# leodd/Lifted-Hybrid-Variational-Inference

Hardware: AMD Instinct MI355X
Metric: lbp_sweeps_per_sec_10M_edge_hybrid_mrf (higher is better)
Workload: dtype f64

## Files before the change

include/lhvi.h:

```cpp
#ifndef LHVI_H
#define LHVI_H

#include <stddef.h>
#include <stdint.h>

#ifdef __cplusplus
extern "C" {
#endif

#define LHVI_ABI_VERSION 26
#define LHVI_MAX_ARITY 6

#define LHVI_OK 0
#define LHVI_E_ARG (-1)
#define LHVI_E_LAUNCH (-2)
#define LHVI_E_UNSUPPORTED (-3)
#define LHVI_E_NODEVICE (-4)
#define LHVI_E_NOT_PD (-5)

#define LHVI_POT_GENERIC 0
#define LHVI_POT_TABLE 1
#define LHVI_POT_GAUSSIAN 2
#define LHVI_POT_QUADRATIC 3
#define LHVI_POT_HYBRID_QUADRATIC 4
#define LHVI_POT_LINEAR_GAUSSIAN 5
#define LHVI_POT_X2 6
#define LHVI_POT_XY 7
#define LHVI_POT_MLN 8
#define LHVI_POT_MLN_HARD 9
#define LHVI_POT_IMAGE_NODE 10
#define LHVI_POT_IMAGE_EDGE 11

typedef struct lhvi_graph {
    int32_t V, F, E, nnz;
    const int32_t* fac_ptr;
    const int32_t* edge_var;
    const int32_t* edge_fac;
    const int32_t* edge_canon;
    const int32_t* var_ptr;
    const int32_t* var_edge;
    const double* edge_count;
    const int32_t* fac_pot;
    const double* var_value;
    const int32_t* var_dom;
    const double* var_mult;
    const double* fac_mult;
    int32_t D;
    const int32_t* dom_cont;
    const double* dom_lo;
    const double* dom_hi;
    const int32_t* dom_ptr;
    const double* dom_val;
    const double* edge_value;
    const int32_t* slot_var;
    const int32_t* hub_vars;
    int32_t n_hubs;
} lhvi_graph_t;
#define LHVI_HUB_DEGREE 64

typedef struct lhvi_pots {
    int32_t P;
    const int32_t* kind;
    const int32_t* off;
    const double* param;
    int32_t interpreted;
} lhvi_pots_t;

int lhvi_version(void);
const char* lhvi_strerror(int code);
int lhvi_last_hip_error(void);
int lhvi_device_count(void);


int lhvi_gabp_init(const lhvi_graph_t* g, double* f2v, double* v2f, void* stream);
int lhvi_gabp_v2f(const lhvi_graph_t* g, const double* f2v, double* v2f, void* stream);
int lhvi_gabp_f2v(const lhvi_graph_t* g, const lhvi_pots_t* pots, const double* v2f, double* f2v, void* stream);
int lhvi_gabp_run(const lhvi_graph_t* g, const lhvi_pots_t* pots, double* f2v, double* v2f, int iterations, void* stream);
typedef struct lhvi_gabp_plan {
    const int32_t* pslot;
    const int32_t* info;
    const double* count;
    int32_t n_hub_rows;
    const int32_t* rec;
    const double* pot_words;
    const int32_t* seg;
    int32_t n_seg;
} lhvi_gabp_plan_t;
size_t lhvi_gabp_pull_workspace_bytes(const lhvi_graph_t* g);
int lhvi_gabp_pull(const lhvi_graph_t* g, const lhvi_pots_t* pots, const lhvi_gabp_plan_t* plan, const double* v_prev,
                   double* v_next, int first, void* stream);
int lhvi_gabp_run_pull(const lhvi_graph_t* g, const lhvi_pots_t* pots, const lhvi_gabp_plan_t* plan, double* f2v, double* v2f,
                       int iterations, void* ws, size_t ws_bytes, void* stream);

int lhvi_gabp_graph_create(const lhvi_graph_t* g, const lhvi_pots_t* pots, const lhvi_gabp_plan_t* plan, double* f2v, double* v2f,
                           double* mu_var, int iterations, void* ws, size_t ws_bytes, void** handle_out);
int lhvi_gabp_graph_launch(void* handle, void* stream);
int lhvi_gabp_graph_destroy(void* handle);

int lhvi_gabp_marginals(const lhvi_graph_t* g, const double* f2v, double* mu_var, void* stream);

size_t lhvi_log_likelihood_workspace_bytes(const lhvi_graph_t* g);
int lhvi_log_likelihood(const lhvi_graph_t* g, const lhvi_pots_t* pots, const double* x, double* out, void* ws, size_t ws_bytes,
                        void* stream);


#define LHVI_PBP_EP 1u
#define LHVI_PBP_EPBP_DISCRETE 2u
#define LHVI_PBP_SKIP_TERMS 16u
#define LHVI_PBP_LEAVE_ROOM 256u
#define LHVI_PBP_CQ 512u
#define LHVI_PBP_BOUNDARY_TOTALS 2048u
#define LHVI_PBP_NO_UNIQ 4096u
#define LHVI_PBP_V2F_RECORDS 8192u
#define LHVI_PBP_WIDE_PAIRS 16384u
#define LHVI_PBP_SHARE_CUS 32768u
#define LHVI_PBP_NO_GRID 128u
#define LHVI_PBP_FUSED_RECORDS16 131072u
#define LHVI_PBP_F2V_HEAVY 262144u
#define LHVI_PBP_F2V_SMALL 524288u
#define LHVI_PBP_F2V_PAIR 1048576u
#define LHVI_PBP_F2V_FAST 2097152u
#define LHVI_PBP_F2V_CQ 4194304u
#define LHVI_PBP_F2V_GENERIC 8388608u
#define LHVI_PBP_F2V_ALL (LHVI_PBP_F2V_HEAVY | LHVI_PBP_F2V_SMALL | LHVI_PBP_F2V_PAIR | LHVI_PBP_F2V_FAST | LHVI_PBP_F2V_CQ | LHVI_PBP_F2V_GENERIC)
#define LHVI_PBP_POW2_GROUPS 65536u

typedef struct lhvi_pbp {
    int32_t n;
    int32_t T;
    uint32_t flags;
    double var_threshold;
    double max_log_value;
    const double* particles;
    const double* old_particles;
    const int32_t* np;
    const uint8_t* uniq;
    const double* q;
    const int32_t* fast_edges;
    int32_t n_fast;
    const int32_t* generic_edges;
    int32_t n_generic;
    int32_t generic_pts_log2;
    const void* fast_desc;
    const void* heavy_desc;
    int32_t n_heavy;
    const void* light_desc;
    int32_t n_light;
    const int32_t* bslot;
    const int32_t* brow_ptr;
    const int64_t* brow_off;
    const int32_t* brow_peer;
    const double* recv;
    int32_t rank;
    const double* var_degree;
    int32_t var_lo, var_hi;
    uint32_t* f2v_ticket;
    const int32_t* prop_desc;
    int32_t n_prop_desc;
    const void* pair_desc;
    int32_t n_pair;
    const void* cq_desc;
    int32_t n_cq;
    const int32_t* v2f_wide;
    int32_t n_v2f_wide;
    const int32_t* v2f_narrow;
    int32_t n_v2f_narrow;
    const int32_t* v2f_hub;
    int32_t n_v2f_hub;
    const int32_t* v2f_mid16;
    int32_t n_v2f_mid16;
    const int32_t* v2f_mid32;
    int32_t n_v2f_mid32;
    const int32_t* prop_hub;
    int32_t n_prop_hub;
    double* prop_partial;
    const int32_t* resample_vars;
    int32_t n_resample_vars;
    const void* small16_desc;
    int32_t n_small16;
    const void* small32_desc;
    int32_t n_small32;
    const int64_t* halo_off;
    double* halo_buf;
} lhvi_pbp_t;

#define LHVI_PBP_DESC_BYTES 128
#define LHVI_PBP_TICKET_WORDS 16
#define LHVI_PBP_TICKET_COUNTERS 8
int lhvi_pbp_describe(const lhvi_graph_t* g, const lhvi_pots_t* pots, const lhvi_pbp_t* s, const int32_t* edges, int32_t count,
                      void* desc_out, void* stream);
int lhvi_pbp_describe_cq(const lhvi_graph_t* g, const lhvi_pots_t* pots, const lhvi_pbp_t* s, const int32_t* edges, int32_t count,
                         void* desc_out, void* stream);
int lhvi_pbp_var_sum(const lhvi_graph_t* g, const lhvi_pbp_t* s, const double* f2v, double* out, void* stream);
int lhvi_pbp_domain_grid(const lhvi_graph_t* g, const lhvi_pbp_t* s, double* x, void* stream);
int lhvi_pbp_refine_grid(const lhvi_graph_t* g, const lhvi_pbp_t* s, const double* logb, double* x, double* best, double* best_val,
                         void* stream);
int lhvi_debug_exp(const double* x, double* y, int64_t n, void* stream);
int lhvi_debug_exp_acc(const double* x, const double* c, double* y, int64_t n, void* stream);
int lhvi_debug_exp_acc_floor(const double* x, const double* c, double* y, int64_t n, void* stream);
int lhvi_debug_log(const double* x, double* y, int64_t n, int32_t which, void* stream);

int lhvi_pbp_classify(const lhvi_graph_t* g, const lhvi_pots_t* pots, const lhvi_pbp_t* s, uint8_t* edge_class, void* stream);

int lhvi_pbp_uniq(const lhvi_graph_t* g, int32_t n, const double* particles, const int32_t* np, uint8_t* uniq, void* stream);
int lhvi_pbp_v2f(const lhvi_graph_t* g, const lhvi_pbp_t* s, const double* f2v, double* v2f, void* stream);
int lhvi_pbp_f2v(const lhvi_graph_t* g, const lhvi_pots_t* pots, const lhvi_pbp_t* s, const double* v2f, double* f2v, void* stream);
int lhvi_pbp_proposal(const lhvi_graph_t* g, const lhvi_pbp_t* s, const double* f2v, double* eta, double* q, void* stream);
int lhvi_pbp_proposal_partial(const lhvi_graph_t* g, const lhvi_pbp_t* s, const double* f2v, double* eta, double* ph, void* stream);
int lhvi_pbp_proposal_finish(const lhvi_graph_t* g, const lhvi_pbp_t* s, const double* ph, double* q, void* stream);
int lhvi_pbp_boundary_pack(const lhvi_graph_t* g, const lhvi_pbp_t* s, const double* f2v, const double* ph, int32_t nb,
                           const int32_t* bvars, double* send, void* stream);
int lhvi_pbp_boundary_reduce(int32_t n_items, const int32_t* width, const int32_t* src_ptr, const int64_t* src_off,
                             const int32_t* dst_ptr, const int64_t* dst_off, const double* in, double* out, void* stream);
int lhvi_pbp_init(const lhvi_graph_t* g, const lhvi_pbp_t* s, double* eta, double* q, double* f2v, double* v2f, void* stream);
int lhvi_pbp_resample(const lhvi_graph_t* g, const lhvi_pbp_t* s, const int64_t* var_gid, uint64_t seed, uint32_t iteration, double* particles_out, void* stream);
int lhvi_pbp_edge_points(const lhvi_graph_t* g, const lhvi_pots_t* pots, const lhvi_pbp_t* s, const double* v2f,
                         int32_t nq, const int32_t* qedge, int32_t npts, const double* x, double* out, void* stream);
int lhvi_pbp_resample_uniq(const lhvi_graph_t* g, const lhvi_pbp_t* s, const int64_t* var_gid, uint64_t seed, uint32_t iteration,
                           double* particles_out, uint8_t* uniq_out, void* stream);
int lhvi_pbp_belief_points(const lhvi_graph_t* g, const lhvi_pots_t* pots, const lhvi_pbp_t* s, const double* v2f,
                           int32_t nq, const int32_t* qvar, int32_t npts, const double* x, double* out, void* stream);
int lhvi_pbp_var_fused(const lhvi_graph_t* g, const lhvi_pbp_t* s, const double* f2v, double* v2f, double* eta, double* q,
                       const int64_t* var_gid, uint64_t seed, uint32_t iteration, double* particles_out, uint8_t* uniq_out,
                       const int32_t* desc, int32_t n16, int32_t n32_t32, int32_t n32_t64, void* stream);
int lhvi_pbp_var_fused64(const lhvi_graph_t* g, const lhvi_pbp_t* s, const double* f2v, double* v2f, double* eta, double* q,
                         const int64_t* var_gid, uint64_t seed, uint32_t iteration, double* particles_out, uint8_t* uniq_out,
                         const int32_t* desc, int32_t n64_t32, int32_t n64_t64, void* stream);
int lhvi_pbp_quad(const lhvi_graph_t* g, const lhvi_pots_t* pots, const lhvi_pbp_t* s, const double* v2f, int64_t nq,
                  const int32_t* row_var, const int64_t* qptr, const int32_t* qedge, const double* qmult, const double* lo,
                  const double* hi, double epsabs, double epsrel, double* z, double* abserr, int32_t* status, void* stream);
int lhvi_pbp_map_brent(const lhvi_graph_t* g, const lhvi_pots_t* pots, const lhvi_pbp_t* s, const double* v2f, int64_t nq,
                       const int32_t* row_var, const int64_t* qptr, const int32_t* qedge, const double* qmult, double xtol,
                       int32_t maxfun, double* xout, double* fout, int32_t* nfev, void* stream);
int lhvi_pbp_kl(const lhvi_graph_t* g, const lhvi_pots_t* pots, const lhvi_pbp_t* s, const double* v2f, int64_t nq,
                const int32_t* row_var, const int64_t* qptr, const int32_t* qedge, const double* qmult, const double* logz,
                int32_t Kp, const double* wp, const double* mup, const double* varp, const double* a, const double* b,
                double epsabs, double epsrel, double* kl, double* abserr, int32_t* status, int32_t* neval, void* stream);

int lhvi_pbp_halo_pack(const double* v2f, int32_t n, int32_t n_rows, const int32_t* row_edge, const int64_t* row_off,
                       const int32_t* row_width, const double* q, int32_t n_q, const int32_t* q_var, const int64_t* q_off,
                       double* out, void* stream);
int lhvi_pbp_halo_unpack(const double* in, int32_t n, int32_t n_rows, const int32_t* row_edge, const int64_t* row_off,
                         const int32_t* row_width, double* v2f, int32_t n_q, const int32_t* q_var, const int64_t* q_off,
                         double* q, void* stream);


typedef struct lhvi_vi {
    int32_t K;
    int32_t T;
    int32_t Dmax;
    int32_t quirks;
    const double* gh_x;
    const double* gh_w;
    const double* w;
    const double* eta_c;
    const double* eta_d;
    const double* obs_var;
    const double* var_N;
    const int32_t* fac_list;
    int32_t n_cc, n_grp3, n_grp6, n_rest3, n_rest6;
    int32_t n_tiny;
    int32_t tiny_par_words;
    const int32_t* edge_axis;
} lhvi_vi_t;
#define LHVI_VI_GAUSSIAN_PDF 2
#define LHVI_VI_GROUP_SLOTS 24
#define LHVI_VI_GROUP_COMP 48
#define LHVI_VI_TINY_NODES 32

// ... 273 lines not shown
```

lifted-hybrid-variational-inference_amd/csrc/pbp.hip:

```cpp
#include "common.hpp"
#include "potential.hpp"
#include "fastmath.hpp"
#include "cq.hpp"
#include "gk21.hpp"

namespace lhvi {

__device__ __forceinline__ double wave_sum(double v) { return dpp_wave_reduce(v, SumOp()); }
__device__ __forceinline__ double wave_max(double v) { return dpp_wave_reduce(v, MaxOp()); }
__device__ __forceinline__ int wave_sum_i(int v) {
#pragma unroll
    for (int off = 32; off > 0; off >>= 1) v += __shfl_xor(v, off);
    return v;
}

constexpr double PAD_LOG_TERM = -6.0e5;

__host__ __device__ __forceinline__ int var_first(const lhvi_pbp_t& s) { return s.var_hi > s.var_lo ? s.var_lo : 0; }
__host__ __device__ __forceinline__ int var_limit(const lhvi_graph_t& g, const lhvi_pbp_t& s) { return s.var_hi > s.var_lo ? s.var_hi : g.V; }

__device__ __forceinline__ double norm_pdf_std(double x, double mu, double sig) {
    const double u = (x - mu) / sig;
    return exp(-u * u * 0.5) / (2.506628274631 * sig);
}
// ... 739 lines not shown
        item = nxt;
    }
};

struct HeavyData { double y, m, x0, x1; };

#ifndef LHVI_HEAVY_BLOCK
#define LHVI_HEAVY_BLOCK 256
#endif
#ifndef LHVI_HEAVY_WAVES
#define LHVI_HEAVY_WAVES 7
#endif
#ifndef LHVI_HEAVY_UNROLL
#define LHVI_HEAVY_UNROLL 4
#endif
constexpr int HEAVY_BLOCK = LHVI_HEAVY_BLOCK;

template <int CTRL, int BANK>
__device__ __forceinline__ double dpp_into(double old, double src) {
    const int lo = __builtin_amdgcn_update_dpp(__double2loint(old), __double2loint(src), CTRL, 0xf, BANK, false);
    const int hi = __builtin_amdgcn_update_dpp(__double2hiint(old), __double2hiint(src), CTRL, 0xf, BANK, false);
    return __hiloint2double(hi, lo);
}
__device__ __forceinline__ double fold_bit5(double x, double y) {
    auto lo = __builtin_amdgcn_permlane32_swap(__double2loint(x), __double2loint(y), false, false);
    auto hi = __builtin_amdgcn_permlane32_swap(__double2hiint(x), __double2hiint(y), false, false);
    return __hiloint2double(hi[0], lo[0]) + __hiloint2double(hi[1], lo[1]);
}
__device__ __forceinline__ double fold_bit4(double x, double y) {
    auto lo = __builtin_amdgcn_permlane16_swap(__double2loint(x), __double2loint(y), false, false);
    auto hi = __builtin_amdgcn_permlane16_swap(__double2hiint(x), __double2hiint(y), false, false);
    return __hiloint2double(hi[0], lo[0]) + __hiloint2double(hi[1], lo[1]);
}
__device__ __forceinline__ double fold_bit3(double x, double y) {
    return dpp_into<0x128, 0x3>(y, x) + dpp_into<0x128, 0xc>(x, y);
}
__device__ __forceinline__ double fold_bit2(double x, double y) {
    return dpp_into<0x104, 0x5>(y, x) + dpp_into<0x114, 0xa>(x, y);
}
__device__ __forceinline__ double fold_bit1(double x, double y, bool bit1) {
    const double send = bit1 ? x : y, keep = bit1 ? y : x;
    return keep + dpp_move<0x4e>(send);
}
__device__ __forceinline__ double fold_bit0(double x) { return x + dpp_move<0xb1>(x); }

__device__ __forceinline__ int grid_owned_point(int lane) {
    return 8 * (2 * ((lane >> 1) & 1) + ((lane >> 2) & 1)) + 4 * ((lane >> 3) & 1) + 2 * ((lane >> 4) & 1) + ((lane >> 5) & 1);
}

__device__ __forceinline__ double grid_sums32(double& g, double q, int lane) {
    double z[4];
#pragma unroll
    for (int bt = 0; bt < 4; ++bt) {
        double v[8];
#pragma unroll
        for (int i = 0; i < 8; ++i) { v[i] = g; g *= q; }
        const double u0 = fold_bit4(fold_bit5(v[0], v[1]), fold_bit5(v[2], v[3]));
        const double u1 = fold_bit4(fold_bit5(v[4], v[5]), fold_bit5(v[6], v[7]));
        z[bt] = fold_bit3(u0, u1);
    }
    return fold_bit0(fold_bit1(fold_bit2(z[0], z[1]), fold_bit2(z[2], z[3]), (lane >> 1) & 1));
}
__device__ __forceinline__ double fold_bit0_xy(double x, double y, bool bit0) {
    const double send = bit0 ? x : y, keep = bit0 ? y : x;
    return keep + dpp_move<0xb1>(send);
}
template <int W, typename Step>
__device__ __forceinline__ void small_grid_sums32(Step&& step , int lane, double& s0, double& s1) {
    double z[4];
    const bool b1 = (lane >> 1) & 1, b0 = lane & 1;
#pragma unroll
    for (int bt = 0; bt < 4; ++bt) {
        double v[8];
#pragma unroll
        for (int i = 0; i < 8; ++i) v[i] = step();
        if (W == 32) {
            const double u0 = fold_bit3(fold_bit4(v[0], v[1]), fold_bit4(v[2], v[3]));
            const double u1 = fold_bit3(fold_bit4(v[4], v[5]), fold_bit4(v[6], v[7]));
            z[bt] = fold_bit2(u0, u1);
        } else {
            const double u0 = fold_bit2(fold_bit3(v[0], v[1]), fold_bit3(v[2], v[3]));
            const double u1 = fold_bit2(fold_bit3(v[4], v[5]), fold_bit3(v[6], v[7]));
            z[bt] = fold_bit1(u0, u1, b1);
        }
    }
    if (W == 32) { s0 = fold_bit0_xy(fold_bit1(z[0], z[1], b1), fold_bit1(z[2], z[3], b1), b0); s1 = 0.0; }
    else { s0 = fold_bit0_xy(z[0], z[1], b0); s1 = fold_bit0_xy(z[2], z[3], b0); }
}
template <int W>
__device__ __forceinline__ int small_grid_point(int lane, int k) {
    if (W == 32) return 8 * (((lane >> 1) & 1) + 2 * (lane & 1)) + ((lane >> 4) & 1) + 2 * ((lane >> 3) & 1) + 4 * ((lane >> 2) & 1);
    return 16 * k + 8 * (lane & 1) + ((lane >> 3) & 1) + 2 * ((lane >> 2) & 1) + 4 * ((lane >> 1) & 1);
}
template <int W>
struct SmallGeom {
    static constexpr int G = WAVE / W;
    static constexpr bool POW2 = W == 16 || W == 32;
    static constexpr int L = POW2 ? 0 : (W % 4 == 0 ? 2 : 1);
    static constexpr int OWN = (8 + W - 1) / W;
    static constexpr int P = W >> L;
    static constexpr int R = (32 + W - 1) / W;
    static constexpr int BUF_AB = POW2 ? 0 : G * 4 * P;
};
template <int W, typename Step, typename Emit>
__device__ __forceinline__ void small_grid_sums_lds(Step&& step , int lane, int grp, int gl, bool lane_ok,
                                                    double* __restrict__ buf, Emit&& emit ) {
    using Geo = SmallGeom<W>;
    constexpr int L = Geo::L, P = Geo::P;
    const bool b0 = lane & 1, b1 = (lane >> 1) & 1;
#pragma unroll
    for (int bt = 0; bt < 4; ++bt) {
        double v[8];
#pragma unroll
        for (int i = 0; i < 8; ++i) v[i] = step();
        static_assert(L >= 1, "an even width: the fold over lane ^ 1 stays inside the group");
        {
            double w[4];
#pragma unroll
            for (int m = 0; m < 4; ++m) w[m] = fold_bit0_xy(v[2 * m], v[2 * m + 1], b0);
            if (L == 1) {
                if (lane_ok) {
#pragma unroll
                    for (int m = 0; m < 4; ++m) buf[(grp * 8 + 2 * m + (int)b0) * P + (gl >> 1)] = w[m];
                }
            } else {
                const double u0 = fold_bit1(w[0], w[1], b1), u1 = fold_bit1(w[2], w[3], b1);
                if (lane_ok) {
                    buf[(grp * 8 + 2 * (int)b1 + (int)b0) * P + (gl >> 2)] = u0;
                    buf[(grp * 8 + 4 + 2 * (int)b1 + (int)b0) * P + (gl >> 2)] = u1;
                }
            }
        }
        LHVI_WAVE_SYNC();
        int first = gl - (8 * bt) % W;
        if (first < 0) first += W;
#pragma unroll
        for (int o = 0; o < Geo::OWN; ++o) {
            const int off = first + o * W;
            const bool has = off < 8;
            const double* __restrict__ row = buf + (grp * 8 + (has ? off : 0)) * P;
            double sum = row[0];
#pragma unroll
            for (int k = 1; k < P; ++k) sum += row[k];
            emit(has, 8 * bt + off, sum);
        }
        LHVI_WAVE_SYNC();
    }
}
constexpr int GRID_MIN_NJ = 24;
constexpr double GRID_MAX_EXPONENT = 600.0;
constexpr int GRID_MAX_T = 128;
__device__ __forceinline__ bool grid_eligible(int uniform_grid, int nj, int T) { return uniform_grid && nj >= GRID_MIN_NJ && T <= GRID_MAX_T; }

__device__ __forceinline__ int round_log2_width(int rem) {
    int lw = 6;
    if (rem <= 32) { lw = 0; while ((1 << lw) < rem) ++lw; }
    return lw;
}

struct HeavyArgs {
    int32_t n, T;
    uint32_t flags;
    const double* particles;
    const double* old_particles;
    const double* dom_val;
    uint32_t* f2v_ticket;
    uint32_t* stats;
};
template <typename T>
__device__ __forceinline__ T heavy_arg_reload(size_t offset) {
    auto p = (const __attribute__((address_space(4))) char*)__builtin_amdgcn_kernarg_segment_ptr();
    asm volatile("" : "+s"(p));
    return *(const __attribute__((address_space(4))) T*)(p + offset);
}
struct HeavyHead {
    int32_t e, tv, pv, pce, cls, pos, kind, nj, np, T, gb, par_off;
    double pval;
    int32_t type, grid;
};
struct HeavyCoef { double ay, by, c, axy, bx, kx, gx0, gh; };
struct HeavyDesc { HeavyHead h; HeavyCoef k; };
static_assert(sizeof(HeavyDesc) == sizeof(FastDesc) && offsetof(HeavyDesc, k) == offsetof(FastDesc, ay) &&
              offsetof(HeavyHead, pval) == offsetof(FastDesc, pval) && offsetof(HeavyHead, grid) == offsetof(FastDesc, pad) + 4 &&
              offsetof(HeavyCoef, gx0) + offsetof(HeavyDesc, k) == offsetof(FastDesc, pad2), "HeavyDesc is FastDesc in two halves");

template <typename T> using global_ptr = __attribute__((address_space(1))) T*;
template <typename T>
__device__ __forceinline__ global_ptr<T> scalar_row(T* p) { global_ptr<T> q = (global_ptr<T>)p; asm("" : "+s"(q)); return q; }

template <typename T>
__device__ __forceinline__ T row_load(global_ptr<T> row, uint32_t i) { return *(global_ptr<T>)((global_ptr<const char>)row + i * (uint32_t)sizeof(T)); }
template <typename T>
__device__ __forceinline__ void row_store(global_ptr<T> row, uint32_t i, T v) { *(global_ptr<T>)((global_ptr<char>)row + i * (uint32_t)sizeof(T)) = v; }

__device__ __forceinline__ HeavyData heavy_fetch(const HeavyHead& d, const HeavyArgs& s, const double* __restrict__ v2f, int lane) {
    HeavyData h;
    const int n = s.n, np = d.np, npts = grid_eligible(d.grid, d.nj, d.T) ? d.np : d.np + d.T;
    const uint32_t ul = (uint32_t)lane;
    const auto prow = scalar_row(s.particles + (int64_t)d.tv * n);
    const auto grid_row = [&] { return scalar_row(heavy_arg_reload<const double*>(offsetof(HeavyArgs, dom_val)) + d.gb); };
    h.y = d.pval; h.m = 0.0; h.x0 = 0.0; h.x1 = 0.0;
    if (is_hidden(d.pval) && lane < d.nj) {
        h.y = row_load(scalar_row(s.old_particles + (int64_t)d.pv * n), ul);
        h.m = row_load(scalar_row(v2f + (int64_t)d.pce * n), ul);
    }
    if (np == 64 && npts == 64) {
        h.x0 = row_load(prow, ul);
    } else {
        const int pl = lane & ((1 << round_log2_width(npts)) - 1);
        if (pl < npts) h.x0 = pl < np ? row_load(prow, (uint32_t)pl) : row_load(grid_row(), (uint32_t)(pl - np));
    }
    if (npts > 64) {
        const int rem = npts - 64, pl = lane & ((1 << round_log2_width(rem)) - 1), pp = 64 + pl;
        if (pl < rem) h.x1 = pp < np ? row_load(prow, (uint32_t)pp) : row_load(grid_row(), (uint32_t)(pp - np));
    }
    return h;
}

__global__ void __launch_bounds__(HEAVY_BLOCK) __attribute__((amdgpu_waves_per_eu(LHVI_HEAVY_WAVES, LHVI_HEAVY_WAVES))) pbp_f2v_heavy_kernel(HeavyArgs s, const double* __restrict__ v2f,
                                                             double* __restrict__ f2v, const HeavyDesc* __restrict__ descs,
                                                             int nitems) {
    __shared__ AB sh_all[HEAVY_BLOCK / WAVE][WAVE];
    __shared__ double sh_tab[EXP_TAB_N];
    __shared__ LogRec sh_log[LOG_TAB_N];
    load_log_table(sh_log);
    load_exp_table(sh_tab);
    const int wid = __builtin_amdgcn_readfirstlane(threadIdx.x >> 6);
    const int lane = threadIdx.x & 63;
    AB* sh = sh_all[wid];
    const int n = s.n, S = s.n + s.T;
    WorkCursor<8, HEAVY_BLOCK / WAVE> cur;
    const auto ticket = [] { return heavy_arg_reload<uint32_t*>(offsetof(HeavyArgs, f2v_ticket)); };
    if (!cur.start(ticket, nitems, lane)) return;
    int n_grid = 0, n_direct = 0;
    struct { int32_t e, nj, np, T, gb, grid; double ay, by, c, axy, bx, kx, gx0, gh; } d;
    HeavyHead hn = descs[cur.item].h;
    HeavyData h = heavy_fetch(hn, s, v2f, lane);
    for (;;) {
        d.e = hn.e; d.nj = hn.nj; d.np = hn.np; d.T = hn.T; d.gb = hn.gb; d.grid = hn.grid;
        {
            const HeavyCoef k = descs[cur.item].k;
            d.ay = k.ay; d.by = k.by; d.c = k.c; d.axy = k.axy; d.bx = k.bx; d.kx = k.kx; d.gx0 = k.gx0; d.gh = k.gh;
        }
        const int nxt = cur.next();
        const bool more = nxt < cur.limit;
        hn = descs[__builtin_amdgcn_readfirstlane(min(nxt, cur.limit - 1))].h;
        const int np = d.np, nj = d.nj;
        const auto out = scalar_row(f2v + (int64_t)d.e * S);
        const double kconst = d.kx;
        const bool eligible = grid_eligible(d.grid, nj, d.T);
        bool grid_path = eligible && !(s.flags & (LHVI_PBP_SKIP_TERMS | LHVI_PBP_NO_GRID));
        AB mine;
        mine.a = PAD_LOG_TERM; mine.b = 0.0;
        LHVI_WAVE_SYNC();
        {
            if (lane < nj) {
                const double y = h.y;
                mine.a = (d.ay * y + d.by) * y + d.c + h.m;
                mine.b = d.axy * y + d.bx;
            }
            AB scaled;
            scaled.a = mine.a * LHVI_EXP_INV_STEP; scaled.b = mine.b * LHVI_EXP_INV_STEP;
            sh[lane] = scaled;
        }
        LHVI_WAVE_SYNC();
        if (grid_path) {
            const double X = fmax(fabs(d.gx0), fabs(fma((double)(d.T - 1), d.gh, d.gx0)));
            const double bound = fma(fabs(mine.b) + fabs(kconst) * X, X, fabs(mine.a));
            grid_path = __ballot(lane < nj && !(bound < GRID_MAX_EXPONENT)) == 0;
            if (grid_path) ++n_grid; else ++n_direct;
        }
        const int npts = eligible ? np : np + d.T;
        const double x0 = h.x0, x1 = h.x1;
        if (more) h = heavy_fetch(hn, s, v2f, lane);
        if (grid_path) {
            double gv = exp_core(fma(mine.b, d.gx0, mine.a), sh_tab);
            const double q = exp_core(mine.b * d.gh, sh_tab);
            for (int t0 = 0; t0 < d.T; t0 += 32) {
                const double sum = grid_sums32(gv, q, lane);
                const int t = t0 + grid_owned_point(lane);
                if (t < d.T && !(lane & 1)) {
                    const double xt = fma((double)t, d.gh, d.gx0);
                    row_store(out, (uint32_t)(n + t), sum > 0.0 ? fma(kconst * xt, xt, log_table(sum, sh_log)) : -700.0);
                }
            }
        } else if (eligible) {
#pragma nounroll
            for (int t0 = 0; t0 < d.T; t0 += 64) {
                const int rem = d.T - t0;
                const int lw = round_log2_width(rem);
                const int width = 1 << lw, split = 64 >> lw, sub = lane >> lw, pl = lane & (width - 1);
                const bool valid = pl < rem;
                const double X1 = valid ? heavy_arg_reload<const double*>(offsetof(HeavyArgs, dom_val))[d.gb + t0 + pl] : 0.0, C = kconst * X1 * X1;
                const int chunk = (s.flags & LHVI_PBP_SKIP_TERMS) ? 0 : (nj + split - 1) >> (6 - lw);
                double acc = fast_accumulate_floor<LHVI_HEAVY_UNROLL>(sh + sub * chunk, sh_tab, chunk, X1, C);
                for (int off = width; off < 64; off <<= 1) acc += __shfl_xor(acc, off);
                if (valid && sub == 0) row_store(out, (uint32_t)(n + t0 + pl), acc > 0.0 ? log_table(acc, sh_log) : -700.0);
            }
        }
#pragma nounroll
        for (int r = 0; r < 2; ++r) {
            const int rem = npts - 64 * r;
            if (rem <= 0) break;
            const int lw = round_log2_width(rem);
            const int width = 1 << lw, split = 64 >> lw, sub = lane >> lw, pl = lane & (width - 1);
            const int p = 64 * r + pl;
            const bool valid = pl < rem;
            const double xv = r == 0 ? x0 : x1;
            const double X1 = valid ? xv : 0.0, C = kconst * X1 * X1;
            const int chunk = (s.flags & LHVI_PBP_SKIP_TERMS) ? 0 : (nj + split - 1) >> (6 - lw);
            double acc = fast_accumulate_floor<LHVI_HEAVY_UNROLL>(sh + sub * chunk, sh_tab, chunk, X1, C);
            for (int off = width; off < 64; off <<= 1) acc += __shfl_xor(acc, off);
            if (valid && sub == 0) row_store(out, (uint32_t)(p < np ? p : n + (p - np)), acc > 0.0 ? log_table(acc, sh_log) : -700.0);
        }
        if (!more) break;
        cur.advance(nxt, lane, ticket);
    }
    uint32_t* stats = heavy_arg_reload<uint32_t*>(offsetof(HeavyArgs, stats));
    if (stats && lane == 0) { atomicAdd(stats, (uint32_t)n_grid); atomicAdd(stats + 1, (uint32_t)n_direct); }
}

#ifndef LHVI_SMALL_WAVES
#define LHVI_SMALL_WAVES 6
#endif
#ifndef LHVI_SMALL_WAVES10
#define LHVI_SMALL_WAVES10 5
#endif
#ifndef LHVI_SMALL_WAVES2
#define LHVI_SMALL_WAVES2 5
#endif
template <int W, int PPL = 1>
__global__ void __launch_bounds__(BLOCK) __attribute__((amdgpu_waves_per_eu(PPL == 2 ? LHVI_SMALL_WAVES2 : W == 10 ? LHVI_SMALL_WAVES10 : LHVI_SMALL_WAVES, 8))) pbp_f2v_small_kernel(lhvi_graph_t g, lhvi_pbp_t s, const double* __restrict__ v2f,
                                                            double* __restrict__ f2v, const FastDesc* __restrict__ descs, int nitems) {
    using Geo = SmallGeom<W>;
    constexpr int G = Geo::G;
    constexpr int GS = PPL * W + 1;
    constexpr int SH_AB = G * GS > Geo::BUF_AB ? G * GS : Geo::BUF_AB;
    __shared__ AB sh_all[BLOCK / WAVE][SH_AB];
    __shared__ double sh_tab[EXP_TAB_N];
    __shared__ LogRec sh_log[LOG_TAB_N];
    load_log_table(sh_log);
    load_exp_table(sh_tab);
    const int wid = __builtin_amdgcn_readfirstlane(threadIdx.x >> 6);
    const int lane = threadIdx.x & 63;
    const bool lane_ok = lane < G * W;
    const int grp = lane_ok ? lane / W : G - 1, gl = lane_ok ? lane % W : W - 1;
    AB* sh = sh_all[wid];
    const AB* mine_recs = sh + grp * GS;
    const int n = s.n, S = s.n + s.T;
    const int nsteps = (nitems + G - 1) / G;
    const int nwaves = gridDim.x * (BLOCK / WAVE);
    for (int step = blockIdx.x * (BLOCK / WAVE) + wid; step < nsteps; step += nwaves) {
        const int idx = step * G + grp;
        const bool live = idx < nitems && lane_ok;
        union { FastDesc d; int4 q[sizeof(FastDesc) / 16]; } u;
        {
            const int4* dp = reinterpret_cast<const int4*>(descs + min(idx, nitems - 1));
#pragma unroll
            for (int k = 0; k < (int)(sizeof(FastDesc) / 16); ++k) u.q[k] = dp[k];
        }
        const int touch = reinterpret_cast<const int*>(descs + min((step + nwaves) * G + grp, nitems - 1))[0];
        const FastDesc& d = u.d;
        const int e = d.e, tv = d.tv, nj = d.nj, np = d.np, T = d.T, gb = d.gb;
        const double pval = d.pval, kx = d.kx;
        const int npts = np + T;
        double yl[PPL], ml[PPL];
#pragma unroll
        for (int pp = 0; pp < PPL; ++pp) {
            const int jl = min(gl + pp * W, nj - 1);
            yl[pp] = s.old_particles[(int64_t)d.pv * n + jl]; ml[pp] = v2f[(int64_t)d.pce * n + jl];
        }
        double xs[3];
#pragma unroll
        for (int r = 0; r < 3; ++r) {
            const int p = r * W + gl;
            const double* src = p < np ? s.particles + ((int64_t)tv * n + p) : g.dom_val + (gb + max(min(p - np, T - 1), 0));
            xs[r] = *src;
        }
        const bool hidden_partner = is_hidden(pval);
        double ua[PPL], ub[PPL];
        AB rec[PPL];
#pragma unroll
        for (int pp = 0; pp < PPL; ++pp) {
            const double y = hidden_partner ? yl[pp] : pval, m = hidden_partner ? ml[pp] : 0.0;
            ua[pp] = PAD_LOG_TERM; ub[pp] = 0.0;
            if (gl + pp * W < nj) {
                ua[pp] = (d.ay * y + d.by) * y + d.c + m;
                ub[pp] = d.axy * y + d.bx;
            }
            rec[pp].a = ua[pp] * LHVI_EXP_INV_STEP; rec[pp].b = ub[pp] * LHVI_EXP_INV_STEP;
        }
        const double gx0 = d.pad2[0], gh = d.pad2[1];
        bool gok = false;
        if (d.pad[1] && T <= GRID_MAX_T && !(s.flags & (LHVI_PBP_SKIP_TERMS | LHVI_PBP_NO_GRID))) {
            const double X = fmax(fabs(gx0), fabs(fma((double)(T - 1), gh, gx0)));
            bool mine_bad = false;
#pragma unroll
            for (int pp = 0; pp < PPL; ++pp) {
                const double bound = fma(fabs(ub[pp]) + fabs(kx) * X, X, fabs(ua[pp]));
                mine_bad |= gl + pp * W < nj && !(bound < GRID_MAX_EXPONENT);
            }
            const uint64_t bad = __ballot(mine_bad);
            gok = ((bad >> (grp * W)) & ((1ull << W) - 1)) == 0;
        }
        const int lim = gok ? np : npts;
        const bool any_grid = __ballot(gok && live) != 0;
        int jmax = 0, pmax = 0;
#pragma unroll
        for (int k = 0; k < G; ++k) {
            jmax = max(jmax, __builtin_amdgcn_readlane(nj, k * W));
            pmax = max(pmax, __builtin_amdgcn_readlane(lim, k * W));
        }
        if (s.flags & LHVI_PBP_SKIP_TERMS) jmax = 0;
        double* out = f2v + (int64_t)e * S;
        LHVI_WAVE_SYNC();
        if (lane_ok) {
#pragma unroll
            for (int pp = 0; pp < PPL; ++pp) sh[grp * GS + gl + pp * W] = rec[pp];
        }
        LHVI_WAVE_SYNC();
        asm volatile("" : "+v"(xs[0]), "+v"(xs[1]), "+v"(xs[2]));
#pragma unroll
        for (int r = 0; r < 3; ++r) {
            if (r * W < pmax) {
                const int p = r * W + gl;
                const bool valid = live && p < lim;
                const double x = valid ? xs[r] : 0.0;
                const double acc = fast_accumulate_floor<4, true>(mine_recs, sh_tab, jmax, x, kx * x * x);
                if (valid) out[p < np ? p : n + (p - np)] = acc > 0.0 ? log_table(acc, sh_log) : -700.0;
            }
        }
#pragma unroll 1
        for (int p0 = 3 * W; p0 < pmax; p0 += W) {
            const int p = p0 + gl;
            const bool valid = live && p < lim;
            double x = 0.0;
            if (valid) x = p < np ? s.particles[(int64_t)tv * n + p] : g.dom_val[gb + p - np];
            const double acc = fast_accumulate_floor<4, true>(mine_recs, sh_tab, jmax, x, kx * x * x);
            if (valid) out[p < np ? p : n + (p - np)] = acc > 0.0 ? log_table(acc, sh_log) : -700.0;
        }
        if (any_grid) {
            double gv[PPL], q[PPL];
#pragma unroll
            for (int pp = 0; pp < PPL; ++pp) { gv[pp] = exp_core(fma(ub[pp], gx0, ua[pp]), sh_tab); q[pp] = exp_core(ub[pp] * gh, sh_tab); }
            auto next_value = [&]() {
                double v = gv[0];
                gv[0] *= q[0];
                if constexpr (PPL == 2) { v += gv[1]; gv[1] *= q[1]; }
                return v;
            };
            int tmax = 0;
#pragma unroll
            for (int k = 0; k < G; ++k) tmax = max(tmax, __builtin_amdgcn_readlane(gok ? T : 0, k * W));
#pragma unroll 1
            for (int t0 = 0; t0 < tmax; t0 += 32) {
                if constexpr (Geo::POW2) {
                    double sum[2];
                    small_grid_sums32<W>(next_value, lane, sum[0], sum[1]);
#pragma unroll
                    for (int k = 0; k < (W == 16 ? 2 : 1); ++k) {
                        const int t = t0 + small_grid_point<W>(gl, k);
                        if (live && gok && t < T) {
                            const double xt = fma((double)t, gh, gx0);
                            out[n + t] = sum[k] > 0.0 ? fma(kx * xt, xt, log_table(sum[k], sh_log)) : -700.0;
                        }
                    }
// ... 2022 lines not shown
```

lifted-hybrid-variational-inference_amd/lhvi/_abi.py:

```python
from __future__ import annotations

import ctypes as C
import os

import numpy as np

_HERE = os.path.dirname(os.path.abspath(__file__))
LIB_PATH = os.environ.get('LHVI_LIB') or os.path.join(os.path.dirname(_HERE), 'csrc', 'liblhvi.so')

c_i32p = C.c_void_p
c_f64p = C.c_void_p


class LhviError(RuntimeError):
    pass


class GraphStruct(C.Structure):
    _fields_ = [
        ('V', C.c_int32), ('F', C.c_int32), ('E', C.c_int32), ('nnz', C.c_int32),
        ('fac_ptr', C.c_void_p), ('edge_var', C.c_void_p), ('edge_fac', C.c_void_p), ('edge_canon', C.c_void_p),
        ('var_ptr', C.c_void_p), ('var_edge', C.c_void_p), ('edge_count', C.c_void_p), ('fac_pot', C.c_void_p),
        ('var_value', C.c_void_p), ('var_dom', C.c_void_p), ('var_mult', C.c_void_p), ('fac_mult', C.c_void_p),
        ('D', C.c_int32),
        ('dom_cont', C.c_void_p), ('dom_lo', C.c_void_p), ('dom_hi', C.c_void_p), ('dom_ptr', C.c_void_p),
        ('dom_val', C.c_void_p), ('edge_value', C.c_void_p), ('slot_var', C.c_void_p),
        ('hub_vars', C.c_void_p), ('n_hubs', C.c_int32),
    ]


class GabpPlanStruct(C.Structure):
    _fields_ = [('pslot', C.c_void_p), ('info', C.c_void_p), ('count', C.c_void_p), ('n_hub_rows', C.c_int32), ('rec', C.c_void_p), ('pot_words', C.c_void_p), ('seg', C.c_void_p), ('n_seg', C.c_int32)]


class PotsStruct(C.Structure):
    _fields_ = [('P', C.c_int32), ('kind', C.c_void_p), ('off', C.c_void_p), ('param', C.c_void_p), ('interpreted', C.c_int32)]


class PbpStruct(C.Structure):
    _fields_ = [
        ('n', C.c_int32), ('T', C.c_int32), ('flags', C.c_uint32),
        ('var_threshold', C.c_double), ('max_log_value', C.c_double),
        ('particles', C.c_void_p), ('old_particles', C.c_void_p), ('np', C.c_void_p), ('uniq', C.c_void_p),
        ('q', C.c_void_p),
        ('fast_edges', C.c_void_p), ('n_fast', C.c_int32), ('generic_edges', C.c_void_p), ('n_generic', C.c_int32),
        ('generic_pts_log2', C.c_int32), ('fast_desc', C.c_void_p), ('heavy_desc', C.c_void_p), ('n_heavy', C.c_int32), ('light_desc', C.c_void_p), ('n_light', C.c_int32),
        ('bslot', C.c_void_p), ('brow_ptr', C.c_void_p), ('brow_off', C.c_void_p), ('brow_peer', C.c_void_p),
        ('recv', C.c_void_p), ('rank', C.c_int32), ('var_degree', C.c_void_p),
        ('var_lo', C.c_int32), ('var_hi', C.c_int32),
        ('f2v_ticket', C.c_void_p),
        ('prop_desc', C.c_void_p), ('n_prop_desc', C.c_int32),
        ('pair_desc', C.c_void_p), ('n_pair', C.c_int32),
        ('cq_desc', C.c_void_p), ('n_cq', C.c_int32),
        ('v2f_wide', C.c_void_p), ('n_v2f_wide', C.c_int32), ('v2f_narrow', C.c_void_p), ('n_v2f_narrow', C.c_int32),
        ('v2f_hub', C.c_void_p), ('n_v2f_hub', C.c_int32),
        ('v2f_mid16', C.c_void_p), ('n_v2f_mid16', C.c_int32), ('v2f_mid32', C.c_void_p), ('n_v2f_mid32', C.c_int32),
        ('prop_hub', C.c_void_p), ('n_prop_hub', C.c_int32), ('prop_partial', C.c_void_p),
        ('resample_vars', C.c_void_p), ('n_resample_vars', C.c_int32),
        ('small16_desc', C.c_void_p), ('n_small16', C.c_int32), ('small32_desc', C.c_void_p), ('n_small32', C.c_int32),
        ('halo_off', C.c_void_p), ('halo_buf', C.c_void_p),
    ]


class ViStruct(C.Structure):
    _fields_ = [
        ('K', C.c_int32), ('T', C.c_int32), ('Dmax', C.c_int32), ('quirks', C.c_int32),
        ('gh_x', C.c_void_p), ('gh_w', C.c_void_p), ('w', C.c_void_p), ('eta_c', C.c_void_p), ('eta_d', C.c_void_p),
        ('obs_var', C.c_void_p), ('var_N', C.c_void_p),
        ('fac_list', C.c_void_p), ('n_cc', C.c_int32), ('n_grp3', C.c_int32), ('n_grp6', C.c_int32), ('n_rest3', C.c_int32),
        ('n_rest6', C.c_int32), ('n_tiny', C.c_int32), ('tiny_par_words', C.c_int32), ('edge_axis', C.c_void_p),
    ]


class ViOptStruct(C.Structure):
    _fields_ = [(n, C.c_void_p) for n in ('w_tau', 'w', 'eta_c', 'tau_d', 'eta_d', 'm_w', 's_w', 'm_c', 's_c', 'm_d', 's_d',
                                          'g_w', 'g_c', 'g_d', 'fe')] + \
               [(n, C.c_double) for n in ('lr', 'b1', 'b2', 'eps', 'var_min')] + [('t', C.c_int32)]


PBP_EP = 1
PBP_EPBP_DISCRETE = 2
PBP_SKIP_TERMS = 16
PBP_NO_GRID = 128
PBP_LEAVE_ROOM = 256
PBP_BOUNDARY_TOTALS = 2048
PBP_CQ = 512
PBP_NO_UNIQ = 4096
PBP_V2F_RECORDS = 8192
PBP_WIDE_PAIRS = 16384
PBP_SHARE_CUS = 32768
PBP_POW2_GROUPS = 65536
PBP_FUSED_RECORDS16 = 131072
PBP_F2V_HEAVY = 262144
PBP_F2V_SMALL = 524288
PBP_F2V_PAIR = 1048576
PBP_F2V_FAST = 2097152
PBP_F2V_CQ = 4194304
PBP_F2V_GENERIC = 8388608
PBP_F2V_ALL = PBP_F2V_HEAVY | PBP_F2V_SMALL | PBP_F2V_PAIR | PBP_F2V_FAST | PBP_F2V_CQ | PBP_F2V_GENERIC
ABI_VERSION = 26
PBP_DESC_BYTES = 128
COLOR_HASH, COLOR_SORT = 0, 1
HUB_DEGREE = 64
VI_GROUP_SLOTS, VI_GROUP_COMP, VI_TINY_NODES, VI_TINY_K, VI_TINY_PAR = 24, 48, 32, 2, 3072

class MwsStruct(C.Structure):
    _fields_ = [('T', C.c_int32), ('max_flips', C.c_int32), ('epsilon', C.c_double), ('noise_std', C.c_double),
                ('seed', C.c_uint64), ('try_id', C.c_void_p), ('disc', C.c_void_p), ('n_disc', C.c_int32),
                ('num', C.c_void_p), ('n_num', C.c_int32), ('fac_class', C.c_void_p), ('x', C.c_void_p), ('best_x', C.c_void_p),
                ('cur_score', C.c_void_p), ('best_score', C.c_void_p), ('status', C.c_void_p), ('err_flip', C.c_void_p),
                ('rec_score', C.c_void_p), ('rec_zero', C.c_void_p), ('rec_ticks', C.c_void_p)] + \
               [(n, C.c_void_p) for n in ('rp_init', 'rp_clause', 'rp_walk', 'rp_walk_k', 'rp_noise', 'rp_post', 'out_score',
                                          'out_unsat', 'out_winner', 'out_accept', 'out_val')]


class ExactStruct(C.Structure):
    _fields_ = [('Nd', C.c_int32), ('Nc', C.c_int32), ('M', C.c_int64), ('dstates', C.c_void_p), ('dstride', C.c_void_p),
                ('n_quad', C.c_int32), ('quad_ptr', C.c_void_p), ('quad_desc', C.c_void_p), ('quad_par', C.c_void_p),
                ('n_tab', C.c_int32), ('tab_ptr', C.c_void_p), ('tab_desc', C.c_void_p), ('tab_par', C.c_void_p)]


class GibbsStruct(C.Structure):
    _fields_ = [('ex', ExactStruct), ('dstate_off', C.c_void_p), ('vt_ptr', C.c_void_p), ('vt_fac', C.c_void_p),
                ('vh_ptr', C.c_void_p), ('vh_fac', C.c_void_p), ('n_hyb', C.c_int32), ('hyb_quad', C.c_void_p),
                ('hyb_off', C.c_void_p), ('table_doubles', C.c_int32), ('max_states', C.c_int32), ('table_scratch', C.c_void_p),
                ('disc_block_its', C.c_int32), ('num_burnin', C.c_int32), ('num_samples', C.c_int32), ('seed', C.c_uint64)]


E_NOT_PD = -5
EXACT_MAX_NC = 64
GAUSS_EXACT_NB = 64
GAUSS_CHAIN_MAX_BLOCK = 128

MIX_MAX_K, MIX_TILE, MIX_ROWS = 128, 64, 4
MIX_GAUSSIAN, MIX_VI = 0, 1
GMFIT_MAX_K = 16
GMKL_MAX_PANELS = 1024
GMKL_LOGQ = C.CFUNCTYPE(C.c_double, C.c_double, C.c_int64, C.c_void_p)
VI_GAUSSIAN_PDF = 2
NPVI_MAX_K, NPVI_MAX_SLOTS = 16, 24


class NpviOptStruct(C.Structure):
    _fields_ = [(n, C.c_void_p) for n in ('tau', 'theta_c', 'rho', 'm_tau', 's_tau', 'm_c', 's_c', 'm_rho', 's_rho', 'g_tau', 'g_c',
                                          'g_rho', 'obj', 'w', 'eta_c', 'eta_d', 'mu_lo', 'mu_hi')] + \
               [('lvar_lo', C.c_double), ('lvar_hi', C.c_double), ('var_count', C.c_void_p), ('fac_count', C.c_void_p)] + \
               [(n, C.c_double) for n in ('lr', 'b1', 'b2', 'eps')] + [('t', C.c_int32), ('max_slots', C.c_int32), ('max_arity', C.c_int32)]


class MixStruct(C.Structure):
    _fields_ = [('V', C.c_int32), ('K', C.c_int32), ('Dmax', C.c_int32), ('nstates', C.c_void_p), ('logw', C.c_void_p),
                ('rec', C.c_void_p), ('lpi', C.c_void_p), ('pi', C.c_void_p)]


LBFGSB_FUN = C.CFUNCTYPE(C.c_double, C.POINTER(C.c_double), C.c_void_p)

_G, _P, _S, _VI = C.POINTER(GraphStruct), C.POINTER(PotsStruct), C.POINTER(PbpStruct), C.POINTER(ViStruct)
_GP = C.POINTER(GabpPlanStruct)
_MX = C.POINTER(MixStruct)
_NO = C.POINTER(NpviOptStruct)
_vp, _i32, _i64, _u32, _u64, _f64, _sz = C.c_void_p, C.c_int32, C.c_int64, C.c_uint32, C.c_uint64, C.c_double, C.c_size_t

SIGNATURES = {
    'lhvi_version': (C.c_int, []),
    'lhvi_strerror': (C.c_char_p, [C.c_int]),
    'lhvi_last_hip_error': (C.c_int, []),
    'lhvi_device_count': (C.c_int, []),
    'lhvi_gabp_init': (C.c_int, [_G, _vp, _vp, _vp]),
    'lhvi_gabp_v2f': (C.c_int, [_G, _vp, _vp, _vp]),
    'lhvi_gabp_f2v': (C.c_int, [_G, _P, _vp, _vp, _vp]),
    'lhvi_gabp_run': (C.c_int, [_G, _P, _vp, _vp, C.c_int, _vp]),
    'lhvi_gabp_marginals': (C.c_int, [_G, _vp, _vp, _vp]),
    'lhvi_gabp_pull_workspace_bytes': (C.c_size_t, [_G]),
    'lhvi_gabp_pull': (C.c_int, [_G, _P, _GP, _vp, _vp, C.c_int, _vp]),
    'lhvi_gabp_run_pull': (C.c_int, [_G, _P, _GP, _vp, _vp, C.c_int, _vp, C.c_size_t, _vp]),
    'lhvi_gabp_graph_create': (C.c_int, [_G, _P, _GP, _vp, _vp, _vp, C.c_int, _vp, C.c_size_t, C.POINTER(C.c_void_p)]),
    'lhvi_gabp_graph_launch': (C.c_int, [_vp, _vp]),
    'lhvi_gabp_graph_destroy': (C.c_int, [_vp]),
    'lhvi_pbp_uniq': (C.c_int, [_G, _i32, _vp, _vp, _vp, _vp]),
    'lhvi_pbp_classify': (C.c_int, [_G, _P, _S, _vp, _vp]),
    'lhvi_pbp_describe': (C.c_int, [_G, _P, _S, _vp, _i32, _vp, _vp]),
    'lhvi_pbp_describe_cq': (C.c_int, [_G, _P, _S, _vp, _i32, _vp, _vp]),
    'lhvi_log_likelihood_workspace_bytes': (C.c_size_t, [_G]),
    'lhvi_log_likelihood': (C.c_int, [_G, _P, _vp, _vp, _vp, C.c_size_t, _vp]),
    'lhvi_pbp_var_sum': (C.c_int, [_G, _S, _vp, _vp, _vp]),
    'lhvi_pbp_domain_grid': (C.c_int, [_G, _S, _vp, _vp]),
    'lhvi_pbp_refine_grid': (C.c_int, [_G, _S, _vp, _vp, _vp, _vp, _vp]),
    'lhvi_debug_exp': (C.c_int, [_vp, _vp, _i64, _vp]),
    'lhvi_debug_log': (C.c_int, [_vp, _vp, _i64, C.c_int32, _vp]),
    'lhvi_debug_exp_acc': (C.c_int, [_vp, _vp, _vp, _i64, _vp]),
    'lhvi_debug_exp_acc_floor': (C.c_int, [_vp, _vp, _vp, _i64, _vp]),
    'lhvi_pbp_v2f': (C.c_int, [_G, _S, _vp, _vp, _vp]),
    'lhvi_pbp_f2v': (C.c_int, [_G, _P, _S, _vp, _vp, _vp]),
    'lhvi_pbp_proposal': (C.c_int, [_G, _S, _vp, _vp, _vp, _vp]),
    'lhvi_pbp_proposal_partial': (C.c_int, [_G, _S, _vp, _vp, _vp, _vp]),
    'lhvi_pbp_proposal_finish': (C.c_int, [_G, _S, _vp, _vp, _vp]),
    'lhvi_pbp_boundary_pack': (C.c_int, [_G, _S, _vp, _vp, _i32, _vp, _vp, _vp]),
    'lhvi_pbp_boundary_reduce': (C.c_int, [_i32, _vp, _vp, _vp, _vp, _vp, _vp, _vp, _vp]),
    'lhvi_pbp_halo_pack': (C.c_int, [_vp, _i32, _i32, _vp, _vp, _vp, _vp, _i32, _vp, _vp, _vp, _vp]),
    'lhvi_pbp_halo_unpack': (C.c_int, [_vp, _i32, _i32, _vp, _vp, _vp, _vp, _i32, _vp, _vp, _vp, _vp]),
    'lhvi_pbp_init': (C.c_int, [_G, _S, _vp, _vp, _vp, _vp, _vp]),
    'lhvi_pbp_resample': (C.c_int, [_G, _S, _vp, _u64, _u32, _vp, _vp]),
    'lhvi_pbp_edge_points': (C.c_int, [_G, _P, _S, _vp, _i32, _vp, _i32, _vp, _vp, _vp]),
    'lhvi_pbp_resample_uniq': (C.c_int, [_G, _S, _vp, _u64, _u32, _vp, _vp, _vp]),
    'lhvi_pbp_belief_points': (C.c_int, [_G, _P, _S, _vp, _i32, _vp, _i32, _vp, _vp, _vp]),
    'lhvi_pbp_map_brent': (C.c_int, [_G, _P, _S, _vp, _i64, _vp, _vp, _vp, _vp, _f64, _i32, _vp, _vp, _vp, _vp]),
    'lhvi_pbp_var_fused': (C.c_int, [_G, _S, _vp, _vp, _vp, _vp, _vp, _u64, _u32, _vp, _vp, _vp, _i32, _i32, _i32, _vp]),
    'lhvi_pbp_var_fused64': (C.c_int, [_G, _S, _vp, _vp, _vp, _vp, _vp, _u64, _u32, _vp, _vp, _vp, _i32, _i32, _vp]),
    'lhvi_pbp_quad': (C.c_int, [_G, _P, _S, _vp, _i64, _vp, _vp, _vp, _vp, _vp, _vp, _f64, _f64, _vp, _vp, _vp, _vp]),
    'lhvi_pbp_kl': (C.c_int, [_G, _P, _S, _vp, _i64, _vp, _vp, _vp, _vp, _vp, _i32, _vp, _vp, _vp, _vp, _vp, _f64, _f64, _vp, _vp, _vp, _vp,
                              _vp]),
    'lhvi_vi_workspace_bytes': (_sz, [_G, _VI]),
    'lhvi_vi_grad': (C.c_int, [_G, _P, _VI, _vp, _vp, _vp, _vp, _vp, _sz, _vp]),
    'lhvi_vi_adam_run': (C.c_int, [_G, _P, _VI, C.POINTER(ViOptStruct), _i32, _vp, _vp, _sz, _vp]),
    'lhvi_adam_step': (C.c_int, [_vp, _vp, _vp, _vp, _i64, _i32, _f64, _f64, _f64, _f64, _i32, _f64, _vp]),
    'lhvi_softmax_rows': (C.c_int, [_vp, _vp, _i64, _i32, _i32, _vp]),
    'lhvi_vi_map_bfgs': (C.c_int, [_G, _VI, _i64, _vp, _f64, _i32, _vp, _vp, _vp, _vp, _vp]),
    'lhvi_color_workspace_bytes': (_sz, [_G]),
    'lhvi_color_refine_factors': (C.c_int, [_G, _vp, _vp, _vp, _vp, _vp, _vp, _sz, _i32, _vp]),
    'lhvi_color_refine_rvs': (C.c_int, [_G, _vp, _vp, _vp, _vp, _vp, _sz, _i32, _vp]),
    'lhvi_color_first_members': (C.c_int, [_vp, _i32, _i32, _vp, _vp]),
    'lhvi_color_segment_sums': (C.c_int, [_vp, _vp, _i32, _vp, _vp]),
    'lhvi_mws_init': (C.c_int, [_G, _P, C.POINTER(MwsStruct), _vp]),
    'lhvi_mws_flips': (C.c_int, [_G, _P, C.POINTER(MwsStruct), _i32, _i32, _vp]),
    'lhvi_lbfgsb_host': (C.c_int, [_i32, _vp, LBFGSB_FUN, _vp, _vp, _vp, _vp, _vp]),
    'lhvi_wall_clock_khz': (C.c_int, [_vp]),
    'lhvi_exact_lds_bytes': (_sz, [_i32, _i32, _i32]),
    'lhvi_exact_configs': (C.c_int, [C.POINTER(ExactStruct), _i64, _i64, _i32, _vp, _vp, _vp, _vp, _vp, _vp]),
    'lhvi_exact_normalize': (C.c_int, [_i64, _vp, _vp, _vp, _vp, _vp]),
    'lhvi_exact_marginals': (C.c_int, [C.POINTER(ExactStruct), _i32, _vp, _vp, _vp]),
    'lhvi_exact_mix_prepare': (C.c_int, [_i32, _i64, _vp, _vp, _vp, _vp, _vp]),
    'lhvi_exact_mixture': (C.c_int, [_i32, _i64, _vp, _i32, _vp, _vp, _vp]),
    'lhvi_exact_map_polish': (C.c_int, [_i32, _i64, _vp, _i32, _vp, _vp, _vp, _vp, _i32, _vp, _vp]),
    'lhvi_exact_config_host': (C.c_int, [C.POINTER(ExactStruct), _i64, _vp, _vp, _vp, _vp]),
    'lhvi_gibbs_lds_bytes': (_sz, [_i32, _i32, _i32, _i32]),
    'lhvi_gibbs_init': (C.c_int, [C.POINTER(GibbsStruct), _i64, _vp, _vp]),
    'lhvi_gibbs_run': (C.c_int, [C.POINTER(GibbsStruct), _i64, _i32, _i32, _i32, _vp, _vp, _vp, _vp, _vp, _vp, _vp, _vp, _vp, _vp]),
    'lhvi_gauss_exact_tri_doubles': (_sz, [_i64]),
    'lhvi_gauss_exact_ws_doubles': (_sz, [_i64]),
    'lhvi_gauss_exact_assemble': (C.c_int, [_i64, _i64, _vp, _vp, _vp, _vp, _vp, _vp, _vp, _vp, _vp, _vp]),
    'lhvi_gauss_exact_pack': (C.c_int, [_i64, _vp, _vp, _vp]),
    'lhvi_gauss_exact_factor': (C.c_int, [_i64, _vp, _vp, _vp, _vp, _vp, _vp]),
    'lhvi_gauss_exact_inverse': (C.c_int, [_i64, _vp, _vp, _vp]),
    'lhvi_gauss_exact_moments': (C.c_int, [_i64, _vp, _vp, _vp, _vp, _vp, _vp]),
    'lhvi_gauss_exact_cov': (C.c_int, [_i64, _vp, _i32, _vp, _vp, _vp]),
    'lhvi_gauss_exact_host': (C.c_int, [_i64, _vp, _vp, _vp, _vp, _vp, _vp]),
    'lhvi_gauss_chain_ws_doubles': (_sz, [_i64, _i64, _i64]),
    'lhvi_gauss_chain_solve': (C.c_int, [_i64, _i64, _i64, _vp, _vp, _vp, _vp, _vp, _vp, _vp, _vp, _vp, _vp, _vp]),
    'lhvi_gauss_chain_host': (C.c_int, [_i64, _i64, _i64, _vp, _vp, _vp, _vp, _vp, _vp, _vp, _vp, _vp, _vp]),
    'lhvi_mix_prepare': (C.c_int, [_i32, _i32, _i32, _i32, _vp, _vp, _vp, _vp, _vp, _vp, _vp, _vp]),
    'lhvi_mix_condition_ws_doubles': (_sz, [_i64, _i32, _i32]),
    'lhvi_mix_condition': (C.c_int, [_MX, _i64, _i32, _vp, _vp, _vp, _vp, _vp, _vp, _vp]),
    'lhvi_mix_marginal_map': (C.c_int, [_MX, _i64, _vp, _i32, _vp, _vp, _vp, _i32, _vp, _vp, _vp, _i32, _i32, _vp, _vp, _vp]),
# ... 219 lines not shown
```

Baseline: 70.11.

## Add register-tiled accumulation path for 64-particle heavy factor messages

Adds a specialized path in the heavy factor-to-variable kernel for the case np==64 and npts==64. It uses permlane32 swaps so each lane evaluates two x points against two shared-memory rows per step, with four independent accumulators, and hoists the constant-term exp out of the inner loop. It also sets the rounding mode via s_setreg. The aim is to cut the LDS reads per exp and raise instruction-level parallelism compared with the generic split loop. The new path can be disabled with a new NO_TILE flag and bumps the ABI version.

```diff
diff --git a/include/lhvi.h b/include/lhvi.h
--- a/include/lhvi.h
+++ b/include/lhvi.h
@@ -8,7 +8,7 @@
 extern "C" {
 #endif
 
-#define LHVI_ABI_VERSION 26
+#define LHVI_ABI_VERSION 27
 #define LHVI_MAX_ARITY 6
 
 #define LHVI_OK 0
@@ -115,6 +115,7 @@
 #define LHVI_PBP_WIDE_PAIRS 16384u
 #define LHVI_PBP_SHARE_CUS 32768u
 #define LHVI_PBP_NO_GRID 128u
+#define LHVI_PBP_NO_TILE 1024u
 #define LHVI_PBP_FUSED_RECORDS16 131072u
 #define LHVI_PBP_F2V_HEAVY 262144u
 #define LHVI_PBP_F2V_SMALL 524288u
diff --git a/lifted-hybrid-variational-inference_amd/csrc/pbp.hip b/lifted-hybrid-variational-inference_amd/csrc/pbp.hip
--- a/lifted-hybrid-variational-inference_amd/csrc/pbp.hip
+++ b/lifted-hybrid-variational-inference_amd/csrc/pbp.hip
@@ -915,6 +915,43 @@
 constexpr int GRID_MAX_T = 128;
 __device__ __forceinline__ bool grid_eligible(int uniform_grid, int nj, int T) { return uniform_grid && nj >= GRID_MIN_NJ && T <= GRID_MAX_T; }
 
+__device__ __forceinline__ void gather_halves(double x, double (&v)[2]) {
+    const int xl = __double2loint(x), xh = __double2hiint(x);
+    auto l5 = __builtin_amdgcn_permlane32_swap(xl, xl, false, false);
+    auto h5 = __builtin_amdgcn_permlane32_swap(xh, xh, false, false);
+    v[0] = __hiloint2double(h5[0], l5[0]); v[1] = __hiloint2double(h5[1], l5[1]);
+}
+__device__ __forceinline__ double tile_accumulate_floor(const AB* __restrict__ sh, const double* __restrict__ tab, int steps_, double X1,
+                                                        double kconst, int lane) {
+    const int steps = __builtin_amdgcn_readfirstlane(steps_);
+    const double MAGIC = 6755399441055744.0;
+    double C = kconst * X1 * X1;
+    double kd = fma(C, LHVI_EXP_INV_STEP, MAGIC) - MAGIC;
+    const double magic = 844424930131968.0 + (kd - (double)(24 << LHVI_EXP_TABLE_BITS));
+    double xs[2], ms[2];
+    gather_halves(X1, xs);
+    gather_halves(magic, ms);
+    asm volatile("s_setreg_imm32_b32 hwreg(HW_REG_MODE, 2, 2), 2\n\ts_nop 1" : "+v"(C), "+v"(kd) : : "memory");
+    double r = fma(kd, -LHVI_EXP_STEP_HI, C);
+    r = fma(kd, -LHVI_EXP_STEP_LO, r);
+    double p = fma(r, 1.6666666666666666667e-1, 0.5);
+    p = fma(p, r, 1.0);
+    double sc = fma(p, r, 1.0);
+    double acc[4] = {0.0, 0.0, 0.0, 0.0};
+    const AB* __restrict__ row = sh + 2 * (lane >> 5);
+    for (int i = 0; i < steps; ++i) {
+        const AB r0 = row[4 * i], r1 = row[4 * i + 1];
+#pragma unroll
+        for (int m = 0; m < 2; ++m) {
+            acc[2 * m] = exp_accumulate_floor(acc[2 * m], fma(r0.b, xs[m], r0.a), ms[m], tab);
+            acc[2 * m + 1] = exp_accumulate_floor(acc[2 * m + 1], fma(r1.b, xs[m], r1.a), ms[m], tab);
+        }
+    }
+    double b0 = fold_bit5(acc[0], acc[2]), b1 = fold_bit5(acc[1], acc[3]);
+    asm volatile("s_setreg_imm32_b32 hwreg(HW_REG_MODE, 2, 2), 0\n\ts_nop 1" : "+v"(b0), "+v"(b1), "+v"(sc) : : "memory");
+    return (b0 + b1) * (sc * LHVI_EXPF_SCALE);
+}
+
 __device__ __forceinline__ int round_log2_width(int rem) {
     int lw = 6;
     if (rem <= 32) { lw = 0; while ((1 << lw) < rem) ++lw; }
@@ -1012,7 +1049,9 @@
         const auto out = scalar_row(f2v + (int64_t)d.e * S);
         const double kconst = d.kx;
         const bool eligible = grid_eligible(d.grid, nj, d.T);
-        bool grid_path = eligible && !(s.flags & (LHVI_PBP_SKIP_TERMS | LHVI_PBP_NO_GRID));
+        uint32_t tile_flags = s.flags;
+        asm volatile("" : "+s"(tile_flags));
+        bool grid_path = eligible && !(tile_flags & (LHVI_PBP_SKIP_TERMS | LHVI_PBP_NO_GRID));
         AB mine;
         mine.a = PAD_LOG_TERM; mine.b = 0.0;
         LHVI_WAVE_SYNC();
@@ -1055,12 +1094,17 @@
                 const int width = 1 << lw, split = 64 >> lw, sub = lane >> lw, pl = lane & (width - 1);
                 const bool valid = pl < rem;
                 const double X1 = valid ? heavy_arg_reload<const double*>(offsetof(HeavyArgs, dom_val))[d.gb + t0 + pl] : 0.0, C = kconst * X1 * X1;
-                const int chunk = (s.flags & LHVI_PBP_SKIP_TERMS) ? 0 : (nj + split - 1) >> (6 - lw);
+                const int chunk = (tile_flags & LHVI_PBP_SKIP_TERMS) ? 0 : (nj + split - 1) >> (6 - lw);
                 double acc = fast_accumulate_floor<LHVI_HEAVY_UNROLL>(sh + sub * chunk, sh_tab, chunk, X1, C);
                 for (int off = width; off < 64; off <<= 1) acc += __shfl_xor(acc, off);
                 if (valid && sub == 0) row_store(out, (uint32_t)(n + t0 + pl), acc > 0.0 ? log_table(acc, sh_log) : -700.0);
             }
         }
+        if (np == 64 && npts == 64 && !(tile_flags & LHVI_PBP_NO_TILE)) {
+            const int steps = (tile_flags & LHVI_PBP_SKIP_TERMS) ? 0 : (nj + 3) >> 2;
+            const double acc = tile_accumulate_floor(sh, sh_tab, steps, x0, kconst, lane);
+            row_store(out, (uint32_t)lane, acc > 0.0 ? log_table(acc, sh_log) : -700.0);
+        } else {
 #pragma nounroll
         for (int r = 0; r < 2; ++r) {
             const int rem = npts - 64 * r;
@@ -1071,10 +1115,11 @@
             const bool valid = pl < rem;
             const double xv = r == 0 ? x0 : x1;
             const double X1 = valid ? xv : 0.0, C = kconst * X1 * X1;
-            const int chunk = (s.flags & LHVI_PBP_SKIP_TERMS) ? 0 : (nj + split - 1) >> (6 - lw);
+            const int chunk = (tile_flags & LHVI_PBP_SKIP_TERMS) ? 0 : (nj + split - 1) >> (6 - lw);
             double acc = fast_accumulate_floor<LHVI_HEAVY_UNROLL>(sh + sub * chunk, sh_tab, chunk, X1, C);
             for (int off = width; off < 64; off <<= 1) acc += __shfl_xor(acc, off);
             if (valid && sub == 0) row_store(out, (uint32_t)(p < np ? p : n + (p - np)), acc > 0.0 ? log_table(acc, sh_log) : -700.0);
+        }
         }
         if (!more) break;
         cur.advance(nxt, lane, ticket);
diff --git a/lifted-hybrid-variational-inference_amd/lhvi/_abi.py b/lifted-hybrid-variational-inference_amd/lhvi/_abi.py
--- a/lifted-hybrid-variational-inference_amd/lhvi/_abi.py
+++ b/lifted-hybrid-variational-inference_amd/lhvi/_abi.py
@@ -85,6 +85,7 @@
 PBP_LEAVE_ROOM = 256
 PBP_BOUNDARY_TOTALS = 2048
 PBP_CQ = 512
+PBP_NO_TILE = 1024
 PBP_NO_UNIQ = 4096
 PBP_V2F_RECORDS = 8192
 PBP_WIDE_PAIRS = 16384
@@ -98,7 +99,7 @@
 PBP_F2V_CQ = 4194304
 PBP_F2V_GENERIC = 8388608
 PBP_F2V_ALL = PBP_F2V_HEAVY | PBP_F2V_SMALL | PBP_F2V_PAIR | PBP_F2V_FAST | PBP_F2V_CQ | PBP_F2V_GENERIC
-ABI_VERSION = 26
+ABI_VERSION = 27
 PBP_DESC_BYTES = 128
 COLOR_HASH, COLOR_SORT = 0, 1
 HUB_DEGREE = 64
```

Result: no change. 70.57 (median of 6 runs) (+0.6%).
